# smritip/real-time-audio-sync

Hardware: AMD Instinct MI355X
Metric: aligned chroma frames/sec, batch=64 OTW c=500; path-index match vs CPU ref (higher is better)
Workload: dtype f64 arithmetic, f32 features in HBM

## Files before the change

### real_time_audio_sync_amd/csrc/otw.hip

```cpp
#include <hip/hip_runtime.h>
#include <math.h>
#include <stddef.h>
#include <stdint.h>
#include <stdlib.h>
#include <string.h>
#include <type_traits>

#include "common.h"
#include "cost.h"

namespace rts {

constexpr int kF = 12;
constexpr int kFetch = 8;

struct OtwArgs {
    const void *ref;
    const void *live;
    const int32_t *live_len;
    int32_t *state;
    int32_t *path;
    double *bands;
    long long live_stride;
    int N, c, max_run_count, variant, cost_kind, mode;
    int path_cap, live_cap;
    int ref_f64, live_f64;
    int clamp_len;
    long long *debug;
    int spec;
    double *dense_acc;
    double *dense_cost;
    const long long *ref_first;
    const int32_t *ref_len;
};

struct LiveFromGlobal {};
struct LiveFromGlobalLean {};
template <typename RT> struct RingElem { using type = RT; };
template <> struct RingElem<LiveFromGlobal> { using type = float; };
template <> struct RingElem<LiveFromGlobalLean> { using type = float; };
template <typename RT> constexpr bool kThroughput = std::is_same<RT, LiveFromGlobalLean>::value;
template <typename RT> constexpr bool kHasLiveRing = !std::is_same<RT, LiveFromGlobal>::value && !kThroughput<RT>;

template <int W, typename RT>
struct OtwLds {
    static constexpr int L = W / 64;
    static constexpr int SWZ = L * 65;
    double R[SWZ];
    double C[SWZ];
    double Dr[2][SWZ];
    double Dc[2][SWZ];
    using E = typename RingElem<RT>::type;
    E livew[kF][kHasLiveRing<RT> ? W : 1];
    double cfresh_min;
    double corner_pa;
    double corner_d;
    int cfresh_idx;
    int rfresh_idx;
    double rfresh_min;
    int plan_t[2], plan_j0[2], plan_flags[2];
    int t, j;
    E refw[kF][W];
};

struct OtwSpecOut {
    double pmin[64];
    int pidx[64];
    double d;
    double d2;
    int k1;
    int flag;
};
template <int W>
struct alignas(16) OtwSpecLds {
    static constexpr int SWZ = (W / 64) * 65;
    double ShR[SWZ];
    double ShC[SWZ];
    OtwSpecOut row[2], col[2];
};

template <int W>
__device__ __forceinline__ int swz(int k) {
    constexpr int L = W / 64;
    const int p = k & (W - 1);
    return (p % L) * 65 + (p / L);
}

__device__ __forceinline__ double dmin(double a, double b) { return (b < a) ? b : a; }

__device__ __forceinline__ double dot_strided12(const double (&x)[kF], const double (&y)[kF]) {
    double t1 = 0.0, t2 = 0.0;
#pragma unroll
    for (int i = 0; i < kF; i += 4) {
// ... 264 lines not shown
#define RTS_STAMP(slot) \
    do {                \
    } while (0)
#define RTS_STAMP2(slot) \
    do {                 \
    } while (0)
#endif

struct OtwCtl {
    int t, j, dir, prev, run_count, status, first, n_path, consumed, rows, cols, truncated, pend_dir;
    int recomputes, pending_col, last_x, last_y, rb_idx, cb_idx;
    int live_hi, ref_hi;
    int spec_valid;
    int ri, ci;
    double cA, cU, cL;
    long long cells;
    double rb_min, cb_min;
    double pfl0, pfl1, pfr0, pfr1;
};

struct OtwEnv {
    int b, lane, c, N, live_len, live_cap, euclid, variant, mode, max_run_count, path_cap, live_f64, ref_f64;
    long long live_base;
    const void *live, *ref;
    int32_t *path;
    bool deferred_update;
};

constexpr int kPlanRow = 1, kPlanCol = 2, kPlanStop = 4, kPlanExit = 8;
constexpr int kPlanHit = 16;
constexpr int kPlanRi = 32, kPlanCi = 64;
constexpr int kPlanHitIf = 128;

__device__ __forceinline__ double otw_load_feat(const void *base, int is_f64, long long idx) {
    return is_f64 ? reinterpret_cast<const double *>(base)[idx] : (double)reinterpret_cast<const float *>(base)[idx];
}

__device__ __forceinline__ void otw_prefetch_live(OtwCtl &k, const OtwEnv &e) {
    const int i0 = e.lane, i1 = e.lane + 64;
    const int f0 = k.live_hi + 1 + i0 / kF, f1 = k.live_hi + 1 + i1 / kF;
    if (f0 < e.live_len) k.pfl0 = otw_load_feat(e.live, e.live_f64, e.live_base + (long long)f0 * kF + i0 % kF);
    if (i1 < kFetch * kF && f1 < e.live_len)
        k.pfl1 = otw_load_feat(e.live, e.live_f64, e.live_base + (long long)f1 * kF + i1 % kF);
}
__device__ __forceinline__ void otw_prefetch_ref(OtwCtl &k, const OtwEnv &e) {
    const int i0 = e.lane, i1 = e.lane + 64;
    const int f0 = k.ref_hi + 1 + i0 / kF, f1 = k.ref_hi + 1 + i1 / kF;
    if (f0 < e.N) k.pfr0 = otw_load_feat(e.ref, e.ref_f64, (long long)f0 * kF + i0 % kF);
    if (i1 < kFetch * kF && f1 < e.N) k.pfr1 = otw_load_feat(e.ref, e.ref_f64, (long long)f1 * kF + i1 % kF);
}
template <int W, typename RT>
__device__ __forceinline__ void otw_commit_live(OtwLds<W, RT> &S, OtwCtl &k, const OtwEnv &e) {
    const int i0 = e.lane, i1 = e.lane + 64;
    const int f0 = k.live_hi + 1 + i0 / kF, f1 = k.live_hi + 1 + i1 / kF;
    if (f0 < e.live_len) S.livew[i0 % kF][f0 & (W - 1)] = (typename RingElem<RT>::type)k.pfl0;
    if (i1 < kFetch * kF && f1 < e.live_len) S.livew[i1 % kF][f1 & (W - 1)] = (typename RingElem<RT>::type)k.pfl1;
    k.live_hi = (k.live_hi + kFetch < e.live_len - 1) ? k.live_hi + kFetch : e.live_len - 1;
    otw_prefetch_live(k, e);
}
template <int W, typename RT>
__device__ __forceinline__ void otw_commit_ref(OtwLds<W, RT> &S, OtwCtl &k, const OtwEnv &e) {
    const int i0 = e.lane, i1 = e.lane + 64;
    const int f0 = k.ref_hi + 1 + i0 / kF, f1 = k.ref_hi + 1 + i1 / kF;
    if (f0 < e.N) S.refw[i0 % kF][f0 & (W - 1)] = (typename RingElem<RT>::type)k.pfr0;
    if (i1 < kFetch * kF && f1 < e.N) S.refw[i1 % kF][f1 & (W - 1)] = (typename RingElem<RT>::type)k.pfr1;
    k.ref_hi = (k.ref_hi + kFetch < e.N - 1) ? k.ref_hi + kFetch : e.N - 1;
// ... 144 lines not shown
    else if (y < jj)
        nd = RTS_DIR_ROW;
    else
        nd = RTS_DIR_BOTH;
    if (e.deferred_update) {
        k.pend_dir = nd;
    } else {
        k.run_count = (nd == k.prev) ? k.run_count + 1 : 1;
        if (nd != RTS_DIR_BOTH) k.prev = nd;
    }
    k.dir = nd;
    k.pending_col = (nd == RTS_DIR_COLUMN);
    k.t = tt;
    k.j = jj;
}

template <int W, typename RT>
__device__ __forceinline__ void otw_refill(OtwLds<W, RT> &S, OtwCtl &k, const OtwEnv &e, int need_live, int need_ref,
                                           bool with_ref = true) {
    const int need_l = (need_live < e.live_len - 1) ? need_live : e.live_len - 1;
    if (need_l > k.live_hi) otw_commit_live<W, RT>(S, k, e);
    if (with_ref) {
        const int need_r = (need_ref < e.N - 1) ? need_ref : e.N - 1;
        if (need_r > k.ref_hi) otw_commit_ref<W, RT>(S, k, e);
    }
}

struct OtwPlan {
    int t, j0, flags;
};

template <int W, typename RT>
__device__ __forceinline__ OtwPlan otw_make_plan(OtwLds<W, RT> &S, OtwCtl &k, const OtwEnv &e, bool spec = false,
                                                 int slot = 0) {
    int flags = 0, pt = k.t;
    if (k.status != RTS_RUNNING) {
        flags = kPlanExit;
    } else if (k.pending_col) {
        flags = kPlanCol;
    } else if (k.t + 1 >= e.live_len) {
        if (e.mode == RTS_MODE_SET_LIVE) k.t = k.t + 1;
        flags = kPlanExit;
    } else if (k.t + 1 >= e.live_cap) {
        k.status = RTS_LIVE_OVERFLOW;
        k.t = e.live_len - 1;
        k.consumed = e.live_len;
        flags = kPlanExit;
    } else {
        pt = k.t + 1;
        flags = kPlanRow | ((k.dir != RTS_DIR_ROW) ? kPlanCol : 0);
    }
    if ((flags & kPlanCol) && k.j + 1 >= e.N) flags |= kPlanStop;
    if (spec) {
        const bool both = flags == (kPlanRow | kPlanCol);
        const bool both_ok = both && k.t <= e.c - 2 && k.j <= e.c - 2;
        if (k.spec_valid && (flags == kPlanRow || flags == kPlanCol || both_ok)) {
            flags |= kPlanHit;
            if (flags & kPlanRow) k.ri ^= 1;
            if (flags & kPlanCol) k.ci ^= 1;
        } else if (k.spec_valid && both && W >= 128 && k.t - ((k.t - e.c + 1 > 0) ? k.t - e.c + 1 : 0) >= 2) {
            flags |= kPlanHitIf;
        }
        flags |= (k.ri ? kPlanRi : 0) | (k.ci ? kPlanCi : 0);
    }
    if (e.lane == 0) {
        S.plan_t[slot] = pt;
        S.plan_j0[slot] = k.j;
        S.plan_flags[slot] = flags;
        if (flags & kPlanExit) {
            S.t = k.t;
            S.j = k.j;
        }
    }
    if constexpr (kHasLiveRing<RT>) {
        if (!spec && !(flags & kPlanExit)) {
            const int jn_p = k.j + ((flags & kPlanCol) ? 1 : 0);
            otw_refill<W, RT>(S, k, e, pt + 1, jn_p + 1);
        }
    }
    OtwPlan p;
    p.t = pt;
    p.j0 = k.j;
    p.flags = flags;
    return p;
}

template <int W, bool DENSE, typename RT>
__device__ __forceinline__ void otw_row_strip(double *R, const OtwArgs &a, const OtwEnv &e, const double *Dr,
                                              int pt, int j0, int jn, double sentinel, double &rf_min, int &rf_idx) {
    const int c = e.c;
    const int k1r = (j0 - c + 1 > 0) ? j0 - c + 1 : 0, nr = j0 - k1r + 1;
    const double x_in = (k1r > 0) ? sentinel : (double)INFINITY;
    const int lo_arg = (jn - c + 1 > 0) ? jn - c + 1 : 0;
    const long long dro = ((long long)e.b * e.live_cap + pt) * e.N + k1r;
    strip_chain<W, DENSE>(Dr, R, R, k1r, nr, x_in, e.lane, lo_arg, rf_min, rf_idx, DENSE ? a.dense_acc + dro : nullptr,
                          DENSE ? a.dense_cost + dro : nullptr, 1);
    if (e.lane == 0 && k1r > 0) R[swz<W>(k1r - 1)] = sentinel;
}

template <int W, bool DENSE, typename RT>
__device__ __forceinline__ void otw_col_strip(OtwLds<W, RT> &S, double *C, const OtwArgs &a, const OtwEnv &e,
// ... 430 lines not shown
    o.row_fresh = is_row;
    o.col_fresh = !is_row;
    o.rf_min = o.cf_min = smin;
    o.rf_idx = o.cf_idx = sidx;
    o.row_corner = o.col_corner = true;
    o.rc = o.cc = cl;
    o.stop = false;
    return o;
}

#ifdef RTS_OTW_FULL_BARRIER
#define RTS_STEP_BARRIER() __syncthreads()
#else
#define RTS_STEP_BARRIER() ::rts::lds_barrier()
#endif

template <int W, int NW, bool DENSE, typename RT, bool SPEC>
__global__ void __launch_bounds__(64 * NW) __attribute__((amdgpu_waves_per_eu(kThroughput<RT> ? 6 : 1)))
otw_advance_kernel(OtwArgs a) {
    static_assert(!SPEC || (NW >= 8 && !DENSE), "the pipelined kernel needs 8 waves and no dense mirror");
    constexpr int NT = 64 * NW;
    constexpr int HW0 = SPEC ? 3 : (NW >= 4) ? 2 : 0;
    constexpr int NHELP = 64 * (NW - HW0);
#if defined(RTS_OTW_STAMPS) && RTS_OTW_STAMPS == 1
    long long stamp_sum[16] = {0, 0, 0, 0, 0, 0, 0, 0, 0, 0, 0, 0, 0, 0, 0, 0};
    int stamp_base = 0;
    long long stamp_last = (long long)__builtin_amdgcn_s_memtime();
    __builtin_amdgcn_s_waitcnt(0xC07F);
#endif
#if defined(RTS_OTW_STAMPS) && RTS_OTW_STAMPS == 2
    long long lw_hit = 0, lb_hit = 0, lw_oth = 0, lb_oth = 0, ln_hit = 0, ln_oth = 0, l_last = 0;
    long long lo_work = 0, lo_t0 = 0;
    long long lo_rounds = 0;
#define RTS_ROUNDS_ACC (&lo_rounds)
#define RTS_LW_BEGIN() do { lo_t0 = (long long)__builtin_amdgcn_s_memtime(); __builtin_amdgcn_s_waitcnt(0xC07F); } while (0)
#define RTS_LW_END(hit) do { const long long t_ = (long long)__builtin_amdgcn_s_memtime(); __builtin_amdgcn_s_waitcnt(0xC07F); if (hit) lo_work += t_ - lo_t0; } while (0)
#else
#define RTS_ROUNDS_ACC nullptr
#define RTS_LW_BEGIN() do { } while (0)
#define RTS_LW_END(hit) do { } while (0)
#endif
    extern __shared__ __align__(16) unsigned char smem_raw[];
    OtwLds<W, RT> &S = *reinterpret_cast<OtwLds<W, RT> *>(smem_raw);
    using LdsT = OtwLds<W, RT>;
    constexpr bool kNoLiveRing = !kHasLiveRing<RT>;
    constexpr bool kRefRing = !SPEC && !kNoLiveRing;
    constexpr size_t kSpecOff = (offsetof(LdsT, refw) + 15) & ~(size_t)15;
    OtwSpecLds<W> &SP = *reinterpret_cast<OtwSpecLds<W> *>(smem_raw + kSpecOff);

    const int tid = threadIdx.x;
    const int lane = tid & 63;
    const int wave = __builtin_amdgcn_readfirstlane(tid >> 6);
    const double sentinel = (a.variant == RTS_VARIANT_OTW) ? 1e10 : (double)INFINITY;
    const double inf = INFINITY;
    OtwEnv e;
    e.b = blockIdx.x;
    e.lane = lane;
    e.c = a.c;
    e.euclid = a.cost_kind == RTS_COST_EUCLID;
    e.variant = a.variant;
    e.mode = a.mode;
    e.max_run_count = a.max_run_count;
    e.path_cap = a.path_cap;
    e.live_f64 = a.live_f64;
    e.ref_f64 = a.ref_f64;
    e.live_base = (long long)e.b * a.live_stride * kF;
    e.live = a.live;
    if (a.ref_first) {
        const int nb = a.ref_len[e.b];
        e.N = nb;
        e.live_cap = 2 * nb;
// ... 128 lines not shown
            if (a.mode == RTS_MODE_SET_LIVE)
                otw_decide<W, RT>(S.R, S.C, k, e, 0, 0, false, 0.0, 0, false, 0.0, 0, false, 0.0, false, 0.0, true);
        } else {
            for (int which = 0; which < 2; which++) {
                const int hi = which ? k.t : k.j;
                double vm;
                int im;
                band_argmin<W>(which ? S.C : S.R, (hi - c + 1 > 0) ? hi - c + 1 : 0, hi, lane, vm, im);
                if (which) {
                    k.cb_min = vm;
                    k.cb_idx = im;
                } else {
                    k.rb_min = vm;
                    k.rb_idx = im;
                }
            }
        }
        if (lane == 0) {
            S.t = k.t;
            S.j = k.j;
        }
    }
    __syncthreads();
    int buf = 0;
    OtwPlan pl;
    pl.t = pl.j0 = 0;
    pl.flags = kPlanExit;
    if constexpr (SPEC) {
        otw_costs_prime<W, RT>(S, e, S.t, S.j, tid, NT);
        if (wave == 0) {
            k.cA = rfl(S.R[swz<W>(k.j)]);
            k.cU = (k.t > 0) ? rfl(S.C[swz<W>(k.t - 1)]) : inf;
            k.cL = (k.j > 0) ? rfl(S.R[swz<W>(k.j - 1)]) : inf;
            pl = otw_make_plan<W, RT>(S, k, e, true);
        }
    } else {
        otw_precompute<W, RT>(S, e, S.t, S.j, S.Dr[0], S.Dc[0], tid, NT);
        if (wave == 0) otw_make_plan<W, RT>(S, k, e);
    }
    __syncthreads();

    int sp = 0;
#ifdef RTS_OTW_PRIO_W0
    if constexpr (SPEC) {
        if (wave == 0) __builtin_amdgcn_s_setprio(RTS_OTW_PRIO_W0);
        if (wave == 1 || wave == 2) __builtin_amdgcn_s_setprio(RTS_OTW_PRIO_W12);
    }
#endif
    if constexpr (SPEC) {
        if (wave >= HW0) {
            for (;;) {
                const int pt = __builtin_amdgcn_readfirstlane(S.plan_t[sp]), j0 = __builtin_amdgcn_readfirstlane(S.plan_j0[sp]);
                const int pflags = otw_resolve_plan(__builtin_amdgcn_readfirstlane(S.plan_flags[sp]), pt, c, &SP.col[sp]);
                if (pflags & kPlanExit) break;
                const bool do_row = (pflags & kPlanRow) != 0, do_col = (pflags & kPlanCol) != 0;
                RTS_LW_BEGIN();
                if constexpr (!kNoLiveRing)
                    if (wave == HW0) otw_refill<W, RT>(S, k, e, pt + 3, 0, false);
                if (!(pflags & kPlanHit)) RTS_STEP_BARRIER();
                if (!(pflags & kPlanStop))
                    otw_costs_advance<W, RT>(S, e, pt, j0 + (do_col ? 1 : 0), do_row, do_col, tid - 64 * HW0, NHELP);
                RTS_LW_END(pflags & kPlanHit);
                RTS_STEP_BARRIER();
                sp ^= 1;
            }
        } else if (wave == 1) {
            for (;;) {
                const int pt = __builtin_amdgcn_readfirstlane(S.plan_t[sp]), j0 = __builtin_amdgcn_readfirstlane(S.plan_j0[sp]);
                const int pflags = otw_resolve_plan(__builtin_amdgcn_readfirstlane(S.plan_flags[sp]), pt, c, &SP.col[sp]);
                if (pflags & kPlanExit) break;
                const int jn = j0 + ((pflags & kPlanCol) ? 1 : 0);
                double *R = (pflags & kPlanRi) ? SP.ShR : S.R, *Rsh = (pflags & kPlanRi) ? S.R : SP.ShR;
                RTS_LW_BEGIN();
                if (!(pflags & kPlanHit)) {
                    if ((pflags & (kPlanRow | kPlanCol | kPlanStop)) == (kPlanRow | kPlanCol))
                        otw_col_strip<W, DENSE, RT>(S, (pflags & kPlanCi) ? SP.ShC : S.C, a, e, S.Dc[(j0 + 1) & 1], pt,
                                                    j0 + 1, true, sentinel);
                    RTS_STEP_BARRIER();
                }
                if ((pflags & (kPlanHit | kPlanRow | kPlanCol)) == (kPlanHit | kPlanRow | kPlanCol)) {
                    const double av = otw_last_cell<W>(R, j0, (j0 - c + 1 > 0) ? j0 - c + 1 : 0, Rsh[swz<W>(j0)],
                                                       Rsh[swz<W>(j0 > 0 ? j0 - 1 : 0)], SP.row[sp].d, sentinel);
                    if (lane == 0) R[swz<W>(j0)] = av;
                }
                if (!(pflags & kPlanStop) && pt + 1 < live_len && pt + 1 < e.live_cap)
                    otw_spec_strip<W, false>(S.Dr[(pt + 1) & 1], R, Rsh, jn, c, lane, sentinel, &SP.row[sp ^ 1], RTS_ROUNDS_ACC);
                RTS_LW_END(pflags & kPlanHit);
                RTS_STEP_BARRIER();
                sp ^= 1;
            }
        } else if (wave == 2) {
            for (;;) {
                const int pt = __builtin_amdgcn_readfirstlane(S.plan_t[sp]), j0 = __builtin_amdgcn_readfirstlane(S.plan_j0[sp]);
                const int pflags = otw_resolve_plan(__builtin_amdgcn_readfirstlane(S.plan_flags[sp]), pt, c, &SP.col[sp]);
                if (pflags & kPlanExit) break;
                const int jn = j0 + ((pflags & kPlanCol) ? 1 : 0);
                double *C = (pflags & kPlanCi) ? SP.ShC : S.C, *Csh = (pflags & kPlanCi) ? S.C : SP.ShC;
                RTS_LW_BEGIN();
                if (!(pflags & kPlanHit)) {
                    if constexpr (kThroughput<RT>) {
                        const bool stop2 = (pflags & kPlanStop) != 0;
                        if (pflags & kPlanRow) {
                            double rf_min = inf;
                            int rf_idx = 0x7fffffff;
                            otw_row_strip<W, DENSE, RT>((pflags & kPlanRi) ? SP.ShR : S.R, a, e, S.Dr[pt & 1], pt, j0, jn, sentinel,
                                                        rf_min, rf_idx);
                            if (lane == 0) {
                                S.rfresh_min = rf_min;
                                S.rfresh_idx = rf_idx;
                            }
                        } else if ((pflags & kPlanCol) && !stop2) {
                            otw_col_strip<W, DENSE, RT>(S, C, a, e, S.Dc[jn & 1], pt, jn, false, sentinel);
                        }
                    }
                    RTS_STEP_BARRIER();
                }
                bool drop = false;
                if ((pflags & (kPlanHit | kPlanRow | kPlanCol)) == (kPlanHit | kPlanRow | kPlanCol)) {
                    const int t0 = pt - 1;
                    const double bv = otw_last_cell<W>(C, t0, (pt - c + 1 > 0) ? pt - c + 1 : 0, Csh[swz<W>(t0)],
                                                       Csh[swz<W>(t0 > 0 ? t0 - 1 : 0)], SP.col[sp].d, sentinel);
                    if (lane == 0) C[swz<W>(t0)] = bv;
                    drop = pt >= c;
                }
                if (!(pflags & kPlanStop) && jn + 1 < N)
                    otw_spec_strip<W, true>(S.Dc[(jn + 1) & 1], C, Csh, pt, c, lane, sentinel, &SP.col[sp ^ 1], RTS_ROUNDS_ACC, drop);
                RTS_LW_END(pflags & kPlanHit);
                RTS_STEP_BARRIER();
                sp ^= 1;
            }
        } else {
#if defined(RTS_OTW_STAMPS) && RTS_OTW_STAMPS == 2
            l_last = (long long)__builtin_amdgcn_s_memtime();
            __builtin_amdgcn_s_waitcnt(0xC07F);
#define RTS_W0_STEP_END(hit)                                              \
    do {                                                                  \
        const long long t0_ = (long long)__builtin_amdgcn_s_memtime();    \
        __builtin_amdgcn_s_waitcnt(0xC07F);                               \
        RTS_STEP_BARRIER();                                               \
        const long long t1_ = (long long)__builtin_amdgcn_s_memtime();    \
        __builtin_amdgcn_s_waitcnt(0xC07F);                               \
        if (hit) {                                                        \
            lw_hit += t0_ - l_last;                                       \
            lb_hit += t1_ - t0_;                                          \
            ln_hit += 1;                                                  \
        } else {                                                          \
            lw_oth += t0_ - l_last;                                       \
            lb_oth += t1_ - t0_;                                          \
            ln_oth += 1;                                                  \
        }                                                                 \
        l_last = t1_;                                                     \
    } while (0)
#else
#define RTS_W0_STEP_END(hit) RTS_STEP_BARRIER()
#endif
            int2 *const path_row = reinterpret_cast<int2 *>(e.path) + (size_t)e.b * e.path_cap;
            const auto hit_steps = [&](auto v2_c, auto defer_c) __attribute__((always_inline)) {
                constexpr bool V2 = decltype(v2_c)::value, DEFER = decltype(defer_c)::value;
#define RTS_RFL_CTL(f) k.f = __builtin_amdgcn_readfirstlane(k.f)
                RTS_RFL_CTL(t), RTS_RFL_CTL(j), RTS_RFL_CTL(dir), RTS_RFL_CTL(prev), RTS_RFL_CTL(run_count);
                RTS_RFL_CTL(status), RTS_RFL_CTL(n_path), RTS_RFL_CTL(consumed), RTS_RFL_CTL(rows), RTS_RFL_CTL(cols);
                RTS_RFL_CTL(truncated), RTS_RFL_CTL(pend_dir), RTS_RFL_CTL(pending_col), RTS_RFL_CTL(last_x);
// ... 37 lines not shown
                    const double prev = (n > 0) ? prev_raw : ((k1 > 0) ? sentinel : inf);
                    const double diag = (pos > 0) ? (is_row ? k.cL : k.cU) + 2 * d : inf;
                    const double cl = vmin(vmin(k.cA + d, diag), prev + d);
                    if (lane == 0) {
                        band[swz<W>(pos)] = cl;
                        other[swz<W>(is_row ? pt : jn)] = cl;
                    }
                    if (is_row) {
                        k.rows += 1;
                        k.consumed = pt + 1;
                        k.cU = k.cA;
                        k.cL = prev;
                    } else {
                        k.cols += 1;
                        k.cL = k.cA;
                        k.cU = prev;
                    }
                    k.cA = cl;
                    k.cells += n + 1;
                    RTS_STAMP(3);
                    double rmin = is_row ? smin : k.rb_min, cmin = is_row ? k.cb_min : smin;
                    int ridx = is_row ? sidx : k.rb_idx, cidx = is_row ? k.cb_idx : sidx;
                    const bool r_new = cl < rmin, c_new = cl < cmin;
                    rmin = r_new ? cl : rmin;
                    ridx = r_new ? jn : ridx;
                    cmin = c_new ? cl : cmin;
                    cidx = c_new ? pt : cidx;
                    k.rb_min = rmin;
                    k.rb_idx = ridx;
                    k.cb_min = cmin;
                    k.cb_idx = cidx;
                    const bool rlt = rmin < cmin;
                    const int x = rlt ? pt : cidx, y = rlt ? ridx : jn;
                    bool append = true;
                    if constexpr (V2) {
                        const int xs = __builtin_amdgcn_readfirstlane(x), ys = __builtin_amdgcn_readfirstlane(y);
                        append = (k.n_path == 0) || (xs > k.last_x && ys >= k.last_y);
                        if (append) {
                            k.last_x = xs;
                            k.last_y = ys;
                        }
                    }
                    if (append) {
                        if (k.n_path < e.path_cap) {
                            if (lane == 0) path_row[k.n_path] = make_int2(x, y);
                        } else {
                            k.truncated = 1;
                        }
                        k.n_path += 1;
                    }
                    int nd = __builtin_amdgcn_readfirstlane((x < pt) ? RTS_DIR_COLUMN : (y < jn) ? RTS_DIR_ROW : RTS_DIR_BOTH);
                    if (pt < c)
                        nd = RTS_DIR_BOTH;
                    else if (k.run_count >= e.max_run_count)
                        nd = (k.prev == RTS_DIR_ROW) ? RTS_DIR_COLUMN : RTS_DIR_ROW;
                    if constexpr (DEFER) {
                        k.pend_dir = nd;
                    } else {
                        k.run_count = (nd == k.prev) ? k.run_count + 1 : 1;
                        if (nd != RTS_DIR_BOTH) k.prev = nd;
                    }
                    k.dir = nd;
                    k.pending_col = (nd == RTS_DIR_COLUMN);
                    k.t = pt;
                    k.j = jn;
                    RTS_STAMP(4);
                    k.spec_valid = 1;
                    pl = otw_make_plan<W, RT>(S, k, e, true, sp ^ 1);
                    RTS_STAMP(5);
                    RTS_W0_STEP_END(true);
                    sp ^= 1;
                }
            };
            for (;;) {
                if constexpr (W == 512 && !kThroughput<RT>) {
                    if (e.variant == RTS_VARIANT_LIVENOTE_V2) {
                        if (e.deferred_update)
                            hit_steps(std::true_type{}, std::true_type{});
                        else
                            hit_steps(std::true_type{}, std::false_type{});
                    } else if (e.deferred_update) {
                        hit_steps(std::false_type{}, std::true_type{});
                    } else {
                        hit_steps(std::false_type{}, std::false_type{});
                    }
                }
                RTS_STAMP2(0);
                const int pt = __builtin_amdgcn_readfirstlane(pl.t), j0 = __builtin_amdgcn_readfirstlane(pl.j0);
                pl.flags = __builtin_amdgcn_readfirstlane(pl.flags);
                const int pflags = otw_resolve_plan(pl.flags, pt, c, &SP.col[sp]);
                if (pflags & kPlanExit) break;
                if ((pl.flags & kPlanHitIf) && (pflags & kPlanHit)) {
                    k.ri ^= 1;
                    k.ci ^= 1;
                }
                const bool do_row = (pflags & kPlanRow) != 0, do_col = (pflags & kPlanCol) != 0;
                const bool stop = (pflags & kPlanStop) != 0;
                const int jn = j0 + (do_col ? 1 : 0);
                double *R = (pflags & kPlanRi) ? SP.ShR : S.R, *C = (pflags & kPlanCi) ? SP.ShC : S.C;
                OtwSettled o;
#if defined(RTS_OTW_STAMPS) && RTS_OTW_STAMPS == 1
                stamp_base = (pflags & kPlanHit) ? 0 : 8;
                if (stamp_base) stamp_sum[14] += 1; else stamp_sum[6] += 1;
#endif
// ... 8 lines not shown
                    if constexpr (!kThroughput<RT>) {
                        if (do_row)
                            otw_row_strip<W, DENSE, RT>(R, a, e, S.Dr[pt & 1], pt, j0, jn, sentinel, rf_min, rf_idx);
                        else if (do_col && !stop)
                            otw_col_strip<W, DENSE, RT>(S, C, a, e, S.Dc[jn & 1], pt, jn, false, sentinel);
                    }
                    RTS_STAMP(9);
                    RTS_STEP_BARRIER();
                    RTS_STAMP(10);
                    if constexpr (kThroughput<RT>) {
                        if (do_row) {
                            rf_min = rfl(S.rfresh_min);
                            rf_idx = __builtin_amdgcn_readfirstlane(S.rfresh_idx);
                        }
                    }
                    const double ld_u = C[swz<W>(pt > 0 ? pt - 1 : 0)], ld_l = R[swz<W>(jn > 0 ? jn - 1 : 0)];
                    o = otw_settle<W, DENSE, RT>(S, R, C, k, a, e, pt, j0, pflags, rf_min, rf_idx, sentinel);
                    k.cA = o.cc;
                    k.cU = (pt > 0) ? rfl(ld_u) : inf;
                    k.cL = (jn > 0) ? rfl(ld_l) : inf;
                }
                RTS_STAMP2(3);
                if (o.stop) {
                    k.status = RTS_STOP_REF_END;
                    k.t = pt;
                    k.j = jn;
                    k.pending_col = 0;
                } else {
                    otw_decide<W, RT>(R, C, k, e, pt, jn, o.row_fresh, o.rf_min, o.rf_idx, o.col_fresh, o.cf_min, o.cf_idx,
                                      o.row_corner, o.rc, o.col_corner, o.cc, false);
                }
                RTS_STAMP2(4);
                k.spec_valid = !o.stop;
                pl = otw_make_plan<W, RT>(S, k, e, true, sp ^ 1);
                RTS_STAMP2(5);
                RTS_W0_STEP_END(pflags & kPlanHit);
                sp ^= 1;
            }
#undef RTS_W0_STEP_END
        }
    } else if constexpr (NW >= 4) {
        if (wave >= HW0) {
            for (;;) {
                const int pt = __builtin_amdgcn_readfirstlane(S.plan_t[0]), j0 = __builtin_amdgcn_readfirstlane(S.plan_j0[0]),
                          pflags = __builtin_amdgcn_readfirstlane(S.plan_flags[0]);
                if (pflags & kPlanExit) break;
                const int jn = j0 + ((pflags & kPlanCol) ? 1 : 0);
                if (!(pflags & kPlanStop))
                    otw_precompute<W, RT>(S, e, pt, jn, S.Dr[buf ^ 1], S.Dc[buf ^ 1], tid - 64 * HW0, NHELP);
                __syncthreads();
                __syncthreads();
                buf ^= 1;
            }
        } else if (wave == 1) {
            for (;;) {
                const int pt = __builtin_amdgcn_readfirstlane(S.plan_t[0]), j0 = __builtin_amdgcn_readfirstlane(S.plan_j0[0]),
                          pflags = __builtin_amdgcn_readfirstlane(S.plan_flags[0]);
                if (pflags & kPlanExit) break;
                if ((pflags & (kPlanRow | kPlanCol | kPlanStop)) == (kPlanRow | kPlanCol))
                    otw_col_strip<W, DENSE, RT>(S, S.C, a, e, S.Dc[buf], pt, j0 + 1, true, sentinel);
                __syncthreads();
                __syncthreads();
                buf ^= 1;
            }
        } else {
            for (;;) {
                RTS_STAMP(0);
                const int pt = __builtin_amdgcn_readfirstlane(S.plan_t[0]), j0 = __builtin_amdgcn_readfirstlane(S.plan_j0[0]),
                          pflags = __builtin_amdgcn_readfirstlane(S.plan_flags[0]);
                if (pflags & kPlanExit) break;
                const bool do_row = (pflags & kPlanRow) != 0, do_col = (pflags & kPlanCol) != 0;
                const bool stop = (pflags & kPlanStop) != 0;
                const int jn = j0 + (do_col ? 1 : 0);
                double rf_min = inf;
                int rf_idx = 0x7fffffff;
                if (do_row)
                    otw_row_strip<W, DENSE, RT>(S.R, a, e, S.Dr[buf], pt, j0, jn, sentinel, rf_min, rf_idx);
                else if (do_col && !stop)
                    otw_col_strip<W, DENSE, RT>(S, S.C, a, e, S.Dc[buf], pt, jn, false, sentinel);
                RTS_STAMP(3);
                __syncthreads();
                RTS_STAMP(5);
                const OtwSettled o = otw_settle<W, DENSE, RT>(S, S.R, S.C, k, a, e, pt, j0, pflags, rf_min, rf_idx, sentinel);
                otw_finish<W, RT>(S, k, e, pt, jn, o);
                RTS_STAMP(8);
                __syncthreads();
                buf ^= 1;
            }
        }
    } else {
        for (;;) {
            RTS_STAMP(0);
            const int pt = __builtin_amdgcn_readfirstlane(S.plan_t[0]), j0 = __builtin_amdgcn_readfirstlane(S.plan_j0[0]),
                      pflags = __builtin_amdgcn_readfirstlane(S.plan_flags[0]);
            if (pflags & kPlanExit) break;
            const bool do_row = (pflags & kPlanRow) != 0, do_col = (pflags & kPlanCol) != 0;
            const bool stop = (pflags & kPlanStop) != 0;
            const int jn = j0 + (do_col ? 1 : 0);
            const int k1r = (j0 - c + 1 > 0) ? j0 - c + 1 : 0, nr = j0 - k1r + 1;
            const int k1c = (pt - c + 1 > 0) ? pt - c + 1 : 0, nc = pt - k1c + 1;
            const bool col_active = do_col && !stop;
            double *Dr = S.Dr[buf], *Dc = S.Dc[buf];

            const int col_wave = (NW > 1 && do_row) ? 1 : 0;
            double rf_min = inf;
            int rf_idx = 0x7fffffff;
            if (do_row && wave == 0) {
                const double x_in = (k1r > 0) ? sentinel : inf;
                const int lo_arg = (jn - c + 1 > 0) ? jn - c + 1 : 0;
                const long long dro = ((long long)e.b * e.live_cap + pt) * N + k1r;
                strip_chain<W, DENSE>(Dr, S.R, S.R, k1r, nr, x_in, lane, lo_arg, rf_min, rf_idx, DENSE ? a.dense_acc + dro : nullptr,
                                      DENSE ? a.dense_cost + dro : nullptr, 1);
                if (lane == 0 && k1r > 0) S.R[swz<W>(k1r - 1)] = sentinel;
            }
            if (col_active && wave == col_wave) {
                const double x_in = (k1c > 0) ? sentinel : inf;
                const int ncc = nc - (do_row ? 1 : 0);
                double fm;
                int fi;
                const double dcorner = Dc[swz<W>(pt)];
                const double pa = (do_row && pt > 0) ? S.C[swz<W>(pt - 1)] + 2 * dcorner : inf;
                const long long dco = ((long long)e.b * e.live_cap + k1c) * N + jn;
                strip_chain<W, DENSE>(Dc, S.C, S.C, k1c, ncc, x_in, lane, k1c, fm, fi, DENSE ? a.dense_acc + dco : nullptr,
                                      DENSE ? a.dense_cost + dco : nullptr, N);
                if (lane == 0) {
                    S.corner_pa = pa;
                    S.corner_d = dcorner;
// ... 43 lines not shown
                        }
                    }
                    if (lane == 0) S.R[swz<W>(jn)] = cl;
                    k.cols += 1;
                    k.cells += nc;
                }
                RTS_STAMP(6);
                if (stop) {
                    k.status = RTS_STOP_REF_END;
                    k.t = pt;
                    k.j = jn;
                    k.pending_col = 0;
                } else {
                    otw_decide<W, RT>(S.R, S.C, k, e, pt, jn, do_row, rf_min, rf_idx, col_active, cf_min, cf_idx, col_active, cl,
                                  do_row, col_active ? cl : row_last, false);
                }
                RTS_STAMP(7);
                otw_make_plan<W, RT>(S, k, e);
            }
            RTS_STAMP(8);
            __syncthreads();
            buf ^= 1;
        }
    }
    __syncthreads();

    {
        int te = S.t, je = S.j;
        const int t_state = te;
        if (te > e.live_cap - 1) te = e.live_cap - 1;
        if (je > N - 1) je = N - 1;
        double *bb = a.bands + (size_t)e.b * 2 * (c + 1);
        const double qnan = __longlong_as_double(0x7ff8000000000000LL);
        const int fl = S.plan_flags[sp];
        const double *Rf = (SPEC && (fl & kPlanRi)) ? SP.ShR : S.R, *Cf = (SPEC && (fl & kPlanCi)) ? SP.ShC : S.C;
        const bool row_missing = (t_state >= e.live_len) && (t_state <= e.live_cap - 1);
        const double sentinel = (e.variant == RTS_VARIANT_OTW) ? 1e10 : (double)INFINITY;
        for (int i = tid; i <= c; i += NT) {
            const int y = je - c + i, x = te - c + i;
            bb[i] = (y >= 0) ? (row_missing ? sentinel : Rf[swz<W>(y)]) : qnan;
            bb[(c + 1) + i] = (x >= 0 && x <= t_state) ? ((row_missing && x == t_state) ? sentinel : Cf[swz<W>(x)]) : qnan;
        }
    }
#if defined(RTS_OTW_STAMPS) && RTS_OTW_STAMPS == 1
    if (tid == 0 && a.debug)
        for (int i = 0; i < 16; i++) a.debug[(size_t)e.b * 16 + i] = stamp_sum[i];
#endif
#if defined(RTS_OTW_STAMPS) && RTS_OTW_STAMPS == 2
    if (tid == 0 && a.debug) {
        long long *dbg = a.debug + (size_t)e.b * 16;
        dbg[0] = lw_hit, dbg[1] = lb_hit, dbg[2] = ln_hit, dbg[3] = lw_oth, dbg[4] = lb_oth, dbg[5] = ln_oth;
    }
    if (a.debug && lane == 0 && wave >= 1 && wave <= 7) a.debug[(size_t)e.b * 16 + 5 + wave] = lo_work;
    if (a.debug && lane == 0 && wave >= 1 && wave <= 2) a.debug[(size_t)e.b * 16 + 12 + wave] = lo_rounds;
#endif
    if (tid == 0) {
        st[RTS_ST_T] = k.t;
        st[RTS_ST_J] = k.j;
        st[RTS_ST_DIRECTION] = e.deferred_update ? RTS_DIR_BOTH : k.dir;
        st[RTS_ST_PREVIOUS] = k.prev;
        st[RTS_ST_RUN_COUNT] = k.run_count;
        st[RTS_ST_STATUS] = k.status;
        st[RTS_ST_FIRST_INSERT] = k.first;
        st[RTS_ST_N_PATH] = k.n_path;
        st[RTS_ST_CONSUMED] = k.consumed;
        st[RTS_ST_ROW_STRIPS] = k.rows;
        st[RTS_ST_COL_STRIPS] = k.cols;
        st[RTS_ST_CELLS_LO] = (int32_t)(uint32_t)(k.cells & 0xffffffffLL);
        st[RTS_ST_CELLS_HI] = (int32_t)(uint32_t)((unsigned long long)k.cells >> 32);
        st[RTS_ST_PATH_TRUNCATED] = k.truncated;
        st[14] = k.pend_dir;
        st[RTS_ST_BAND_RECOMPUTES] = k.recomputes;
    }
}

__device__ __forceinline__ void otw_fresh_state(int32_t *st, int variant) {
    for (int i = 0; i < RTS_STATE_LEN; i++) st[i] = 0;
    st[RTS_ST_DIRECTION] = RTS_DIR_BOTH;
    st[RTS_ST_PREVIOUS] = RTS_DIR_NONE;
    st[RTS_ST_RUN_COUNT] = (variant == RTS_VARIANT_OTW) ? 1 : 0;
    st[RTS_ST_STATUS] = RTS_RUNNING;
    st[RTS_ST_FIRST_INSERT] = 1;
    st[14] = -2;
}

__global__ void otw_reset_kernel(int32_t *state, int B, int variant) {
    const int b = blockIdx.x * blockDim.x + threadIdx.x;
// ... 56 lines not shown
    __syncthreads();
    for (int idx = threadIdx.x; idx < nn * kF; idx += blockDim.x) {
        const int fr = base + idx / kF;
        if (fr < cap) {
            const size_t src = (size_t)b * n_max * kF + idx;
            hist[((size_t)b * cap + fr) * kF + idx % kF] =
                frames_f64 ? reinterpret_cast<const double *>(frames)[src]
                           : (double)reinterpret_cast<const float *>(frames)[src];
        }
    }
    __syncthreads();
    if (threadIdx.x == 0) hist_len[b] = base + (nn > 0 ? nn : 0);
}

}

struct rts_otw {
    const void *ref;
    int ref_dtype, F, N, B, c, max_run_count, variant, cost_kind;
    int W, waves, path_cap;
    int hist_stride;
    int32_t *state;
    int32_t *path;
    double *bands;
    double *hist;
    rts::RefTable refs;
    int32_t *hist_len;
    long long *debug;
    double *dense_acc, *dense_cost;
    int spec;
    int device;
    int cus;
    int tp_from;
    const void *attr_fn[8];
    int src_kind;
    int run_dtype, run_T, run_mode;
    int32_t *rp_state, *rp_path;
    double *rp_bands;
};

namespace rts {

static int ensure_lds_attr(rts_otw *h, const void *fn, size_t smem) {
    for (int k = 0; k < 8; k++)
        if (h->attr_fn[k] == fn) return RTS_OK;
    RTS_HIP(hipFuncSetAttribute(fn, hipFuncAttributeMaxDynamicSharedMemorySize, (int)smem));
    for (int k = 0; k < 8; k++)
        if (!h->attr_fn[k]) {
            h->attr_fn[k] = fn;
            break;
        }
    return RTS_OK;
}

template <int W, int NW, bool DENSE, typename RT, bool SPEC>
static int launch_advance_d(rts_otw *h, const OtwArgs &args, int B, hipStream_t s) {
    using LdsT = OtwLds<W, RT>;
    const size_t smem = SPEC ? ((offsetof(LdsT, refw) + 15) & ~(size_t)15) + sizeof(OtwSpecLds<W>)
                             : (kHasLiveRing<RT> ? sizeof(LdsT) : ((offsetof(LdsT, refw) + 15) & ~(size_t)15));
    const int rc = ensure_lds_attr(h, reinterpret_cast<const void *>(&otw_advance_kernel<W, NW, DENSE, RT, SPEC>), smem);
    if (rc != RTS_OK) return rc;
    hipLaunchKernelGGL((otw_advance_kernel<W, NW, DENSE, RT, SPEC>), dim3(B), dim3(64 * NW), smem, s, args);
    RTS_HIP(hipGetLastError());
    return RTS_OK;
}

// ... 34 lines not shown

static int launch(rts_otw *h, const OtwArgs &args, hipStream_t s) {
    if ((uintptr_t)args.live & 15) return set_error(RTS_ERR_INVALID, "live features must be 16-byte aligned");
    switch (h->W) {
        case 64: return launch_w<64>(h, args, h->B, h->waves, s);
        case 128: return launch_w<128>(h, args, h->B, h->waves, s);
        case 256: return launch_w<256>(h, args, h->B, h->waves, s);
        case 512: return launch_w<512>(h, args, h->B, h->waves, s);
        case 1024: return launch_w<1024>(h, args, h->B, h->waves, s);
        case 2048: return launch_w<2048>(h, args, h->B, h->waves, s);
    }
    return set_error(RTS_ERR_UNSUPPORTED, "no kernel for window %d", h->W);
}

static OtwArgs base_args(const rts_otw *h) {
    OtwArgs a;
    memset(&a, 0, sizeof(a));
    a.ref = h->ref;
    a.state = h->state;
    a.path = h->path;
    a.bands = h->bands;
    a.N = h->N;
    a.c = h->c;
    a.max_run_count = h->max_run_count;
    a.variant = h->variant;
    a.cost_kind = h->cost_kind;
    a.path_cap = h->path_cap;
    a.live_cap = 2 * h->N;
    a.ref_first = h->refs.first;
    a.ref_len = h->refs.len;
    a.ref_f64 = h->ref_dtype == RTS_F64;
    a.debug = h->debug;
    a.spec = h->spec;
    a.dense_acc = h->dense_acc;
    a.dense_cost = h->dense_cost;
    return a;
}

static OtwArgs hist_args(const rts_otw *h) {
    OtwArgs a = base_args(h);
    a.live = h->hist;
    a.live_len = h->hist_len;
    a.live_stride = h->hist_stride;
    a.live_f64 = 1;
    a.mode = RTS_MODE_INSERT_LOOP;
    return a;
}

static int begin_append(rts_otw *h) {
    if (!h->hist) {
        RTS_HIP(hipMalloc((void **)&h->hist, sizeof(double) * kF * (size_t)h->hist_stride * h->B));
    }
    h->src_kind = (h->src_kind == 0 || h->src_kind == 2) ? 2 : 3;
    return RTS_OK;
}

static void fill_dense(const rts_otw *h, double *acc, double *cost, const RestartSel *sel, hipStream_t s) {
    const long long per = (long long)2 * h->N * h->N;
    const double sentinel = (h->variant == RTS_VARIANT_OTW) ? 1e10 : (double)INFINITY;
    if (sel) {
        hipLaunchKernelGGL(otw_fill_sel_kernel, dim3(64, sel->n), dim3(256), 0, s, *sel, acc, per, sentinel);
        hipLaunchKernelGGL(otw_fill_sel_kernel, dim3(64, sel->n), dim3(256), 0, s, *sel, cost, per, -1.0);
    } else {
        hipLaunchKernelGGL(otw_fill_kernel, dim3(2048), dim3(256), 0, s, acc, h->B * per, sentinel);
        hipLaunchKernelGGL(otw_fill_kernel, dim3(2048), dim3(256), 0, s, cost, h->B * per, -1.0);
    }
}

struct OtwKnobs {
    int spec, tp_from;
};
static OtwKnobs otw_knobs() {
    const char *sp = getenv("RTS_OTW_SPEC"), *tp = getenv("RTS_OTW_TP_FROM");
    return {sp ? (atoi(sp) != 0) : 1, tp ? atoi(tp) : 2};
}

static int otw_create(const void *ref_dev, int ref_dtype, int F, int N, int B, int c, int max_run_count, int variant,
                      int cost_kind, const long long *first_host, const int32_t *len_host, rts_otw **out) {
    if (F < 1) return set_error(RTS_ERR_INVALID, "F must be >= 1 (got %d)", F);
    if (F != kF) return set_error(RTS_ERR_UNSUPPORTED, "F must be 12 chroma bins (got %d)", F);
    if (N < 1 || B < 1) return set_error(RTS_ERR_INVALID, "N and B must be >= 1 (got N=%d B=%d)", N, B);
    if (ref_dtype != RTS_F32 && ref_dtype != RTS_F64) return set_error(RTS_ERR_INVALID, "bad ref_dtype %d", ref_dtype);
    if (c < 1) return set_error(RTS_ERR_INVALID, "c must be >= 1 (got %d)", c);
    if (c > 2036)
        return set_error(RTS_ERR_UNSUPPORTED, "band width c=%d exceeds the 2036 cells the LDS-resident kernel holds", c);
    if (max_run_count < 1) return set_error(RTS_ERR_INVALID, "max_run_count must be >= 1");
    if (variant < RTS_VARIANT_OTW || variant > RTS_VARIANT_LIVENOTE_V2)
        return set_error(RTS_ERR_INVALID, "bad variant %d", variant);
    if (cost_kind != RTS_COST_DOT && cost_kind != RTS_COST_EUCLID)
        return set_error(RTS_ERR_INVALID, "bad cost_kind %d", cost_kind);
    if ((long long)N * 3 + 8 > 0x3fffffffLL) return set_error(RTS_ERR_INVALID, "N too large");

    rts_otw *h = (rts_otw *)calloc(1, sizeof(rts_otw));
    if (!h) return set_error(RTS_ERR_INVALID, "out of host memory");
    h->ref = ref_dev;
    h->ref_dtype = ref_dtype;
    h->F = F;
    h->N = N;
    h->B = B;
    h->c = c;
    h->max_run_count = max_run_count;
    h->variant = variant;
    h->cost_kind = cost_kind;
    h->W = 64;
    while (h->W < c + 12) h->W *= 2;
    h->waves = 8;
    const OtwKnobs knobs = otw_knobs();
    h->spec = knobs.spec;
    h->tp_from = knobs.tp_from;
    h->hist_stride = 2 * N;
    h->path_cap = 3 * N + 8;
    hipError_t e;
    if ((e = hipGetDevice(&h->device)) != hipSuccess ||
        (e = hipDeviceGetAttribute(&h->cus, hipDeviceAttributeMultiprocessorCount, h->device)) != hipSuccess) {
        free(h);
        return set_error(RTS_ERR_HIP, "hipGetDevice failed: %s", hipGetErrorString(e));
    }
    if ((e = hipMalloc((void **)&h->state, sizeof(int32_t) * RTS_STATE_LEN * (size_t)B)) != hipSuccess ||
        (e = hipMalloc((void **)&h->path, sizeof(int32_t) * 2 * (size_t)h->path_cap * B)) != hipSuccess ||
        (e = hipMalloc((void **)&h->bands, sizeof(double) * 2 * (size_t)(c + 1) * B)) != hipSuccess ||
        (e = hipMalloc((void **)&h->hist_len, sizeof(int32_t) * (size_t)B)) != hipSuccess ||
        (first_host && (e = ref_table_upload(&h->refs, first_host, len_host, B)) != hipSuccess)) {
        rts_otw_destroy(h);
        return set_error(RTS_ERR_HIP, "hipMalloc failed: %s", hipGetErrorString(e));
    }
    int rc = rts_otw_reset(h, nullptr);
    if (rc != RTS_OK) {
        rts_otw_destroy(h);
        return rc;
    }
    hipLaunchKernelGGL(otw_fill_kernel, dim3(64), dim3(256), 0, nullptr, h->bands, (long long)2 * (c + 1) * B,
                       __builtin_nan(""));
    if ((e = hipGetLastError()) != hipSuccess) {
        rts_otw_destroy(h);
        return set_error(RTS_ERR_HIP, "launch of the band fill failed: %s", hipGetErrorString(e));
    }
    if ((e = hipStreamSynchronize(nullptr)) != hipSuccess) {
        rts_otw_destroy(h);
        return set_error(RTS_ERR_HIP, "hipStreamSynchronize failed: %s", hipGetErrorString(e));
    }
    *out = h;
    return RTS_OK;
// ... 278 lines not shown
```

Baseline: 33.15 million.

## Publish next-step plan early with tagged packed LDS words for helper waves

The plan record moves into a packed, tagged 4-int LDS slot written with two 64-bit volatile stores. Wave 0 now computes the next direction and plan before appending the path entry. Helper waves peek at the next slot before the step barrier and use it directly when the tag matches the step and no conditional hit applies, skipping the post-barrier LDS reads and plan resolution. This aims to shorten the critical path between barriers. The cost is extra speculative LDS reads and a fallback path, and correctness depends on the store and barrier ordering.

After: 32.41 million. 0.978x the previous value.

```diff
diff --git a/real_time_audio_sync_amd/csrc/otw.hip b/real_time_audio_sync_amd/csrc/otw.hip
--- a/real_time_audio_sync_amd/csrc/otw.hip
+++ b/real_time_audio_sync_amd/csrc/otw.hip
@@ -32,6 +32,7 @@
     double *dense_cost;
     const long long *ref_first;
     const int32_t *ref_len;
+    int early_plan;
 };
 
 struct LiveFromGlobal {};
@@ -58,7 +59,7 @@
     int cfresh_idx;
     int rfresh_idx;
     double rfresh_min;
-    int plan_t[2], plan_j0[2], plan_flags[2];
+    alignas(8) int plan[2][4];
     int t, j;
     E refw[kF][W];
 };
@@ -389,6 +390,22 @@
 constexpr int kPlanRi = 32, kPlanCi = 64;
 constexpr int kPlanHitIf = 128;
 
+constexpr int kPlanWordT = 0, kPlanWordJ0 = 1, kPlanWordFlags = 2, kPlanWordTag = 3;
+using OtwPlanWord = __attribute__((address_space(3))) volatile long long;
+__device__ __forceinline__ long long otw_pack2(int lo, int hi) {
+    return (long long)(((unsigned long long)(unsigned)hi << 32) | (unsigned long long)(unsigned)lo);
+}
+__device__ __forceinline__ void otw_plan_store(int *slot, int pt, int j0, int flags, int tag) {
+    OtwPlanWord *w = (OtwPlanWord *)(__attribute__((address_space(3))) int *)slot;
+    w[0] = otw_pack2(pt, j0);
+    w[1] = otw_pack2(flags, tag);
+}
+__device__ __forceinline__ void otw_plan_peek(const int *slot, long long &w_ft, long long &w_tj) {
+    OtwPlanWord *w = (OtwPlanWord *)(__attribute__((address_space(3))) int *)const_cast<int *>(slot);
+    w_ft = w[1];
+    w_tj = w[0];
+}
+
 __device__ __forceinline__ double otw_load_feat(const void *base, int is_f64, long long idx) {
     return is_f64 ? reinterpret_cast<const double *>(base)[idx] : (double)reinterpret_cast<const float *>(base)[idx];
 }
@@ -599,7 +616,7 @@
 
 template <int W, typename RT>
 __device__ __forceinline__ OtwPlan otw_make_plan(OtwLds<W, RT> &S, OtwCtl &k, const OtwEnv &e, bool spec = false,
-                                                 int slot = 0) {
+                                                 int slot = 0, int tag = 0) {
     int flags = 0, pt = k.t;
     if (k.status != RTS_RUNNING) {
         flags = kPlanExit;
@@ -631,9 +648,7 @@
         flags |= (k.ri ? kPlanRi : 0) | (k.ci ? kPlanCi : 0);
     }
     if (e.lane == 0) {
-        S.plan_t[slot] = pt;
-        S.plan_j0[slot] = k.j;
-        S.plan_flags[slot] = flags;
+        otw_plan_store(S.plan[slot], pt, k.j, flags, tag);
         if (flags & kPlanExit) {
             S.t = k.t;
             S.j = k.j;
@@ -1130,11 +1145,14 @@
     long long lw_hit = 0, lb_hit = 0, lw_oth = 0, lb_oth = 0, ln_hit = 0, ln_oth = 0, l_last = 0;
     long long lo_work = 0, lo_t0 = 0;
     long long lo_rounds = 0;
+    long long lo_miss = 0;
 #define RTS_ROUNDS_ACC (&lo_rounds)
+#define RTS_EARLY_MISS() do { lo_miss += 1; } while (0)
 #define RTS_LW_BEGIN() do { lo_t0 = (long long)__builtin_amdgcn_s_memtime(); __builtin_amdgcn_s_waitcnt(0xC07F); } while (0)
 #define RTS_LW_END(hit) do { const long long t_ = (long long)__builtin_amdgcn_s_memtime(); __builtin_amdgcn_s_waitcnt(0xC07F); if (hit) lo_work += t_ - lo_t0; } while (0)
 #else
 #define RTS_ROUNDS_ACC nullptr
+#define RTS_EARLY_MISS() do { } while (0)
 #define RTS_LW_BEGIN() do { } while (0)
 #define RTS_LW_END(hit) do { } while (0)
 #endif
@@ -1329,6 +1347,7 @@
             k.cA = rfl(S.R[swz<W>(k.j)]);
             k.cU = (k.t > 0) ? rfl(S.C[swz<W>(k.t - 1)]) : inf;
             k.cL = (k.j > 0) ? rfl(S.R[swz<W>(k.j - 1)]) : inf;
+            if (lane == 0) S.plan[1][kPlanWordTag] = -1;
             pl = otw_make_plan<W, RT>(S, k, e, true);
         }
     } else {
@@ -1338,6 +1357,9 @@
     __syncthreads();
 
     int sp = 0;
+    constexpr bool kEarly = SPEC && W <= 512 && !kThroughput<RT>;
+    int step = 0;
+    long long ew_ft = otw_pack2(0, -1), ew_tj = 0;
 #ifdef RTS_OTW_PRIO_W0
     if constexpr (SPEC) {
         if (wave == 0) __builtin_amdgcn_s_setprio(RTS_OTW_PRIO_W0);
@@ -1345,10 +1367,29 @@
     }
 #endif
     if constexpr (SPEC) {
+        const auto plan_fetch = [&](int &pt, int &j0, int &pflags) __attribute__((always_inline)) {
+            if constexpr (kEarly) {
+                const int efl = __builtin_amdgcn_readfirstlane((int)ew_ft);
+                const int etag = __builtin_amdgcn_readfirstlane((int)(ew_ft >> 32));
+                if (a.early_plan && etag == step && !(efl & kPlanHitIf)) {
+                    pt = __builtin_amdgcn_readfirstlane((int)ew_tj);
+                    j0 = __builtin_amdgcn_readfirstlane((int)(ew_tj >> 32));
+                    pflags = efl;
+                    return;
+                }
+                RTS_EARLY_MISS();
+            }
+            pt = __builtin_amdgcn_readfirstlane(S.plan[sp][kPlanWordT]);
+            j0 = __builtin_amdgcn_readfirstlane(S.plan[sp][kPlanWordJ0]);
+            pflags = otw_resolve_plan(__builtin_amdgcn_readfirstlane(S.plan[sp][kPlanWordFlags]), pt, c, &SP.col[sp]);
+        };
+        const auto plan_peek = [&]() __attribute__((always_inline)) {
+            if constexpr (kEarly) otw_plan_peek(S.plan[sp ^ 1], ew_ft, ew_tj);
+        };
         if (wave >= HW0) {
             for (;;) {
-                const int pt = __builtin_amdgcn_readfirstlane(S.plan_t[sp]), j0 = __builtin_amdgcn_readfirstlane(S.plan_j0[sp]);
-                const int pflags = otw_resolve_plan(__builtin_amdgcn_readfirstlane(S.plan_flags[sp]), pt, c, &SP.col[sp]);
+                int pt, j0, pflags;
+                plan_fetch(pt, j0, pflags);
                 if (pflags & kPlanExit) break;
                 const bool do_row = (pflags & kPlanRow) != 0, do_col = (pflags & kPlanCol) != 0;
                 RTS_LW_BEGIN();
@@ -1357,14 +1398,16 @@
                 if (!(pflags & kPlanHit)) RTS_STEP_BARRIER();
                 if (!(pflags & kPlanStop))
                     otw_costs_advance<W, RT>(S, e, pt, j0 + (do_col ? 1 : 0), do_row, do_col, tid - 64 * HW0, NHELP);
+                plan_peek();
                 RTS_LW_END(pflags & kPlanHit);
                 RTS_STEP_BARRIER();
                 sp ^= 1;
+                step += 1;
             }
         } else if (wave == 1) {
             for (;;) {
-                const int pt = __builtin_amdgcn_readfirstlane(S.plan_t[sp]), j0 = __builtin_amdgcn_readfirstlane(S.plan_j0[sp]);
-                const int pflags = otw_resolve_plan(__builtin_amdgcn_readfirstlane(S.plan_flags[sp]), pt, c, &SP.col[sp]);
+                int pt, j0, pflags;
+                plan_fetch(pt, j0, pflags);
                 if (pflags & kPlanExit) break;
                 const int jn = j0 + ((pflags & kPlanCol) ? 1 : 0);
                 double *R = (pflags & kPlanRi) ? SP.ShR : S.R, *Rsh = (pflags & kPlanRi) ? S.R : SP.ShR;
@@ -1382,14 +1425,16 @@
                 }
                 if (!(pflags & kPlanStop) && pt + 1 < live_len && pt + 1 < e.live_cap)
                     otw_spec_strip<W, false>(S.Dr[(pt + 1) & 1], R, Rsh, jn, c, lane, sentinel, &SP.row[sp ^ 1], RTS_ROUNDS_ACC);
+                plan_peek();
                 RTS_LW_END(pflags & kPlanHit);
                 RTS_STEP_BARRIER();
                 sp ^= 1;
+                step += 1;
             }
         } else if (wave == 2) {
             for (;;) {
-                const int pt = __builtin_amdgcn_readfirstlane(S.plan_t[sp]), j0 = __builtin_amdgcn_readfirstlane(S.plan_j0[sp]);
-                const int pflags = otw_resolve_plan(__builtin_amdgcn_readfirstlane(S.plan_flags[sp]), pt, c, &SP.col[sp]);
+                int pt, j0, pflags;
+                plan_fetch(pt, j0, pflags);
                 if (pflags & kPlanExit) break;
                 const int jn = j0 + ((pflags & kPlanCol) ? 1 : 0);
                 double *C = (pflags & kPlanCi) ? SP.ShC : S.C, *Csh = (pflags & kPlanCi) ? S.C : SP.ShC;
@@ -1422,9 +1467,11 @@
                 }
                 if (!(pflags & kPlanStop) && jn + 1 < N)
                     otw_spec_strip<W, true>(S.Dc[(jn + 1) & 1], C, Csh, pt, c, lane, sentinel, &SP.col[sp ^ 1], RTS_ROUNDS_ACC, drop);
+                plan_peek();
                 RTS_LW_END(pflags & kPlanHit);
                 RTS_STEP_BARRIER();
                 sp ^= 1;
+                step += 1;
             }
         } else {
 #if defined(RTS_OTW_STAMPS) && RTS_OTW_STAMPS == 2
@@ -1528,6 +1575,24 @@
                     k.cb_idx = cidx;
                     const bool rlt = rmin < cmin;
                     const int x = rlt ? pt : cidx, y = rlt ? ridx : jn;
+                    int nd = __builtin_amdgcn_readfirstlane((x < pt) ? RTS_DIR_COLUMN : (y < jn) ? RTS_DIR_ROW : RTS_DIR_BOTH);
+                    if (pt < c)
+                        nd = RTS_DIR_BOTH;
+                    else if (k.run_count >= e.max_run_count)
+                        nd = (k.prev == RTS_DIR_ROW) ? RTS_DIR_COLUMN : RTS_DIR_ROW;
+                    if constexpr (DEFER) {
+                        k.pend_dir = nd;
+                    } else {
+                        k.run_count = (nd == k.prev) ? k.run_count + 1 : 1;
+                        if (nd != RTS_DIR_BOTH) k.prev = nd;
+                    }
+                    k.dir = nd;
+                    k.pending_col = (nd == RTS_DIR_COLUMN);
+                    k.t = pt;
+                    k.j = jn;
+                    RTS_STAMP(4);
+                    k.spec_valid = 1;
+                    pl = otw_make_plan<W, RT>(S, k, e, true, sp ^ 1, step + 1);
                     bool append = true;
                     if constexpr (V2) {
                         const int xs = __builtin_amdgcn_readfirstlane(x), ys = __builtin_amdgcn_readfirstlane(y);
@@ -1545,27 +1610,10 @@
                         }
                         k.n_path += 1;
                     }
-                    int nd = __builtin_amdgcn_readfirstlane((x < pt) ? RTS_DIR_COLUMN : (y < jn) ? RTS_DIR_ROW : RTS_DIR_BOTH);
-                    if (pt < c)
-                        nd = RTS_DIR_BOTH;
-                    else if (k.run_count >= e.max_run_count)
-                        nd = (k.prev == RTS_DIR_ROW) ? RTS_DIR_COLUMN : RTS_DIR_ROW;
-                    if constexpr (DEFER) {
-                        k.pend_dir = nd;
-                    } else {
-                        k.run_count = (nd == k.prev) ? k.run_count + 1 : 1;
-                        if (nd != RTS_DIR_BOTH) k.prev = nd;
-                    }
-                    k.dir = nd;
-                    k.pending_col = (nd == RTS_DIR_COLUMN);
-                    k.t = pt;
-                    k.j = jn;
-                    RTS_STAMP(4);
-                    k.spec_valid = 1;
-                    pl = otw_make_plan<W, RT>(S, k, e, true, sp ^ 1);
                     RTS_STAMP(5);
                     RTS_W0_STEP_END(true);
                     sp ^= 1;
+                    step += 1;
                 }
             };
             for (;;) {
@@ -1640,18 +1688,19 @@
                 }
                 RTS_STAMP2(4);
                 k.spec_valid = !o.stop;
-                pl = otw_make_plan<W, RT>(S, k, e, true, sp ^ 1);
+                pl = otw_make_plan<W, RT>(S, k, e, true, sp ^ 1, step + 1);
                 RTS_STAMP2(5);
                 RTS_W0_STEP_END(pflags & kPlanHit);
                 sp ^= 1;
+                step += 1;
             }
 #undef RTS_W0_STEP_END
         }
     } else if constexpr (NW >= 4) {
         if (wave >= HW0) {
             for (;;) {
-                const int pt = __builtin_amdgcn_readfirstlane(S.plan_t[0]), j0 = __builtin_amdgcn_readfirstlane(S.plan_j0[0]),
-                          pflags = __builtin_amdgcn_readfirstlane(S.plan_flags[0]);
+                const int pt = __builtin_amdgcn_readfirstlane(S.plan[0][kPlanWordT]), j0 = __builtin_amdgcn_readfirstlane(S.plan[0][kPlanWordJ0]),
+                          pflags = __builtin_amdgcn_readfirstlane(S.plan[0][kPlanWordFlags]);
                 if (pflags & kPlanExit) break;
                 const int jn = j0 + ((pflags & kPlanCol) ? 1 : 0);
                 if (!(pflags & kPlanStop))
@@ -1662,8 +1711,8 @@
             }
         } else if (wave == 1) {
             for (;;) {
-                const int pt = __builtin_amdgcn_readfirstlane(S.plan_t[0]), j0 = __builtin_amdgcn_readfirstlane(S.plan_j0[0]),
-                          pflags = __builtin_amdgcn_readfirstlane(S.plan_flags[0]);
+                const int pt = __builtin_amdgcn_readfirstlane(S.plan[0][kPlanWordT]), j0 = __builtin_amdgcn_readfirstlane(S.plan[0][kPlanWordJ0]),
+                          pflags = __builtin_amdgcn_readfirstlane(S.plan[0][kPlanWordFlags]);
                 if (pflags & kPlanExit) break;
                 if ((pflags & (kPlanRow | kPlanCol | kPlanStop)) == (kPlanRow | kPlanCol))
                     otw_col_strip<W, DENSE, RT>(S, S.C, a, e, S.Dc[buf], pt, j0 + 1, true, sentinel);
@@ -1674,8 +1723,8 @@
         } else {
             for (;;) {
                 RTS_STAMP(0);
-                const int pt = __builtin_amdgcn_readfirstlane(S.plan_t[0]), j0 = __builtin_amdgcn_readfirstlane(S.plan_j0[0]),
-                          pflags = __builtin_amdgcn_readfirstlane(S.plan_flags[0]);
+                const int pt = __builtin_amdgcn_readfirstlane(S.plan[0][kPlanWordT]), j0 = __builtin_amdgcn_readfirstlane(S.plan[0][kPlanWordJ0]),
+                          pflags = __builtin_amdgcn_readfirstlane(S.plan[0][kPlanWordFlags]);
                 if (pflags & kPlanExit) break;
                 const bool do_row = (pflags & kPlanRow) != 0, do_col = (pflags & kPlanCol) != 0;
                 const bool stop = (pflags & kPlanStop) != 0;
@@ -1699,8 +1748,8 @@
     } else {
         for (;;) {
             RTS_STAMP(0);
-            const int pt = __builtin_amdgcn_readfirstlane(S.plan_t[0]), j0 = __builtin_amdgcn_readfirstlane(S.plan_j0[0]),
-                      pflags = __builtin_amdgcn_readfirstlane(S.plan_flags[0]);
+            const int pt = __builtin_amdgcn_readfirstlane(S.plan[0][kPlanWordT]), j0 = __builtin_amdgcn_readfirstlane(S.plan[0][kPlanWordJ0]),
+                      pflags = __builtin_amdgcn_readfirstlane(S.plan[0][kPlanWordFlags]);
             if (pflags & kPlanExit) break;
             const bool do_row = (pflags & kPlanRow) != 0, do_col = (pflags & kPlanCol) != 0;
             const bool stop = (pflags & kPlanStop) != 0;
@@ -1810,7 +1859,7 @@
         if (je > N - 1) je = N - 1;
         double *bb = a.bands + (size_t)e.b * 2 * (c + 1);
         const double qnan = __longlong_as_double(0x7ff8000000000000LL);
-        const int fl = S.plan_flags[sp];
+        const int fl = S.plan[sp][kPlanWordFlags];
         const double *Rf = (SPEC && (fl & kPlanRi)) ? SP.ShR : S.R, *Cf = (SPEC && (fl & kPlanCi)) ? SP.ShC : S.C;
         const bool row_missing = (t_state >= e.live_len) && (t_state <= e.live_cap - 1);
         const double sentinel = (e.variant == RTS_VARIANT_OTW) ? 1e10 : (double)INFINITY;
@@ -1831,6 +1880,7 @@
     }
     if (a.debug && lane == 0 && wave >= 1 && wave <= 7) a.debug[(size_t)e.b * 16 + 5 + wave] = lo_work;
     if (a.debug && lane == 0 && wave >= 1 && wave <= 2) a.debug[(size_t)e.b * 16 + 12 + wave] = lo_rounds;
+    if (a.debug && lane == 0 && wave == 1) a.debug[(size_t)e.b * 16 + 15] = lo_miss;
 #endif
     if (tid == 0) {
         st[RTS_ST_T] = k.t;
@@ -1953,6 +2003,7 @@
     int device;
     int cus;
     int tp_from;
+    int early_plan;
     const void *attr_fn[8];
     int src_kind;
     int run_dtype, run_T, run_mode;
@@ -2053,6 +2104,7 @@
     a.ref_f64 = h->ref_dtype == RTS_F64;
     a.debug = h->debug;
     a.spec = h->spec;
+    a.early_plan = h->early_plan;
     a.dense_acc = h->dense_acc;
     a.dense_cost = h->dense_cost;
     return a;
@@ -2089,11 +2141,11 @@
 }
 
 struct OtwKnobs {
-    int spec, tp_from;
+    int spec, tp_from, early_plan;
 };
 static OtwKnobs otw_knobs() {
-    const char *sp = getenv("RTS_OTW_SPEC"), *tp = getenv("RTS_OTW_TP_FROM");
-    return {sp ? (atoi(sp) != 0) : 1, tp ? atoi(tp) : 2};
+    const char *sp = getenv("RTS_OTW_SPEC"), *tp = getenv("RTS_OTW_TP_FROM"), *ep = getenv("RTS_OTW_EARLY_PLAN");
+    return {sp ? (atoi(sp) != 0) : 1, tp ? atoi(tp) : 2, ep ? (atoi(ep) != 0) : 1};
 }
 
 static int otw_create(const void *ref_dev, int ref_dtype, int F, int N, int B, int c, int max_run_count, int variant,
@@ -2129,6 +2181,7 @@
     const OtwKnobs knobs = otw_knobs();
     h->spec = knobs.spec;
     h->tp_from = knobs.tp_from;
+    h->early_plan = knobs.early_plan;
     h->hist_stride = 2 * N;
     h->path_cap = 3 * N + 8;
     hipError_t e;
```
